# TheProParadox/3dspa_code

Hardware: AMD Instinct MI355X
Metric: train-step tracks/sec (B x N_tracks) at T=150, C=772 (higher is better)
Workload: dtype bf16

## Files before the change

### 3dspa_code_amd/csrc/common.hpp

```cpp
#pragma once
#include <hip/hip_runtime.h>
#include <stdint.h>
#include <string>
#include <vector>

#include "../../include/spa3d.h"
#include "ablate.inc"
#include "gemm_plan.hpp"
#include "score_row.hpp"

#ifndef SPA_F16
#define SPA_F16 0
#endif
#if SPA_F16
#define SPA_NS h_f16
#else
#define SPA_NS h_bf16
#endif
typedef unsigned short bf16_t;

struct DetCfg { float* gbase; long long* shadow; long long n; unsigned* flag; float scale; };
constexpr float DET_ADDEND_MAX = 36028797018963968.f;
constexpr long long DET_SUM_MAX = 1ll << 62;
constexpr int DET_E_MIN = -24, DET_E_MAX = 40;
// ... 117 lines not shown
  bool dry = false, overflow = false;
  void* alloc(int64_t bytes) {
    int64_t a = (off + 255) & ~int64_t(255);
    off = a + bytes;
    if (off > peak) peak = off;
    if (dry) return (void*)(uintptr_t)(0x1000 + a);
    if (off > cap) { overflow = true; return base; }
    return base + a;
  }
  int64_t mark() const { return off; }
  void release(int64_t m) { off = m; }
};

enum { PROF_GEMM_NT = 0, PROF_GEMM_TN = 1, PROF_GEMM_GENERIC = 2, PROF_ATTN_FWD = 3, PROF_ATTN_BWD = 4, PROF_LN_FWD = 5, PROF_LN_BWD = 6,
       PROF_ATTN_Q1 = 7, PROF_EMBED = 8, PROF_NCLS = 9 };
struct ProfRec { int cls; double flops, bytes; hipEvent_t e0, e1; int64_t tag[4] = {0, 0, 0, 0}; };
struct Prof {
  bool on = false;
  std::vector<hipEvent_t> pool; size_t used = 0;
  std::vector<ProfRec> recs;
  hipEvent_t get() {
    if (used == pool.size()) { hipEvent_t e; if (hipEventCreate(&e) != hipSuccess) return nullptr; pool.push_back(e); }
    return pool[used++];
  }
};

struct spa3d_ctx {
  spa3d_config cfg;
  std::vector<Leaf> leaves;
  int64_t nparams = 0;
  std::string err;
  hipStream_t stream = nullptr;
  Arena ar;
  bool dry = false;
  int hip_err = 0;
  GemmPolicy gemm;
  int attn_impl = 0;
  int chunk = 0;
  int query_chunk = 0;
  int track_chunk = 0;
  int ro_share = 1;
  int prune = 1;
  float loss_scale = 1.f;
  void* grad_ev[2] = {nullptr, nullptr};
  int64_t grad_ev_gen[2] = {0, 0};
  bool last_chunk = false;
  const float* loss_scale_state = nullptr;
  double plan_stats[4] = {0, 0, 0, 0};
  int attn_bwd_mode = 0;
  int qkv_attn = 0;
  int det_grads = 0;
  const DetCfg* det = nullptr;
  std::vector<int32_t> cnt_n, cnt_q; bool has_cnt_n = false, has_cnt_q = false; int cnt_B = 0;
  int poison = 0;
  Prof prof;
};

inline void apply_attn_impl(spa3d_ctx* c, int v) {
  c->attn_impl = v == 1 ? 1 : (v >= 2 ? 2 : 0);
  c->attn_bwd_mode = v == 3 ? 2 : (v == 4 ? 3 : 0);
  c->qkv_attn = v == 6;
}

template <typename F> inline int64_t arena_peak(spa3d_ctx* c, F&& body) {
  const Arena saved = c->ar; const bool sd = c->dry;
  c->ar = Arena(); c->ar.dry = true; c->dry = true;
  body();
  const int64_t peak = c->ar.peak;
  c->ar = saved; c->dry = sd;
  return peak;
}
template <typename F> inline int sized_call(spa3d_ctx* c, const char* what, int64_t need, void* ws, int64_t ws_bytes, void* stream, F&& body) {
  if (!ws || ws_bytes < need) { c->err = std::string(what) + ": workspace too small: need " + std::to_string(need) + " bytes"; return SPA3D_ERR_ARG; }
  c->stream = (hipStream_t)stream; c->dry = false;
  c->ar = Arena(); c->ar.base = (char*)ws; c->ar.cap = ws_bytes;
  body();
  if (c->ar.overflow) { c->err = "internal: arena overflow"; return SPA3D_ERR_WORKSPACE; }
  return c->hip_err ? SPA3D_ERR_HIP : SPA3D_OK;
}
inline bool counts_fit_batch(spa3d_ctx* c, int B) {
  if (c->cnt_B == B) return true;
  c->err = "counts were set for B = " + std::to_string(c->cnt_B) + ", this batch has B = " + std::to_string(B);
  return false;
}
inline const int32_t* checked_query_counts(spa3d_ctx* c, int B, int Q) {
  if (!counts_fit_batch(c, B)) return nullptr;
  for (int i = 0; i < B; ++i)
    if (c->cnt_q[i] < 0 || c->cnt_q[i] > Q) {
      c->err = "query_count[" + std::to_string(i) + "] = " + std::to_string(c->cnt_q[i]) + " is outside [0, Q = " + std::to_string(Q) + "]";
      return nullptr;
    }
  return c->cnt_q.data();
}
template <typename F> inline void for_each_live_span(const int32_t* cq, int64_t B, int64_t Q, F&& f) {
  if (!cq) { f((int64_t)0, B * Q); return; }
  for (int64_t i = 0; i < B; ++i) f(i * Q, (int64_t)cq[i]);
}

struct ProfScope {
  spa3d_ctx* c; ProfRec r; bool on;
  ProfScope(spa3d_ctx* c_, int cls, double flops, double bytes) : c(c_), on(c_->prof.on && !c_->dry) {
    if (!on) return;
    r.cls = cls; r.flops = flops; r.bytes = bytes; r.e0 = c->prof.get(); r.e1 = c->prof.get();
    if (!r.e0 || !r.e1) { on = false; return; }
    (void)hipEventRecord(r.e0, c->stream);
  }
// ... 127 lines not shown
```

### 3dspa_code_amd/csrc/gemm_fast.hip

```cpp
#include "common.hpp"
#include "tn_args.hpp"

namespace SPA_NS {

typedef __attribute__((ext_vector_type(4))) float f32x4;
typedef __attribute__((ext_vector_type(16))) float f32x16;
typedef mfma16x8 bf16x8;
typedef __attribute__((ext_vector_type(4))) unsigned short u16x4;

#define GLDS16(gptr, lptr) \
  __builtin_amdgcn_global_load_lds((const __attribute__((address_space(1))) void*)(gptr), (__attribute__((address_space(3))) void*)(lptr), 16, 0, 0)
#define GLDS16_NT(gptr, lptr) \
  __builtin_amdgcn_global_load_lds((const __attribute__((address_space(1))) void*)(gptr), (__attribute__((address_space(3))) void*)(lptr), 16, 0, 2)

__device__ __forceinline__ void glds16_s(const void* base_uniform, unsigned off, const void* lds_dst) {
  const unsigned l = (unsigned)(uintptr_t)lds_dst;
  asm volatile("s_mov_b32 m0, %2\n\ts_nop 0\n\tglobal_load_lds_dwordx4 %0, %1" ::"v"(off), "s"(base_uniform), "s"(l) : "memory", "m0");
}

struct NtArgs {
  const bf16_t* A; const bf16_t* Bt; void* C;
  int64_t M; int N; int K; int64_t lda, ldb, ldc;
  const float* bias; const bf16_t* aux; bf16_t* pre_out; int epi; int out_f32; int accumulate; float alpha;
  int tiles_m, tiles_n, crow_group, crow_skip;
#if SPA3D_ABL_NT
  int ablate;
#endif
  const bf16_t* A2; int64_t lda2; int K1; const int32_t* arow_idx; const int32_t* crow_idx; const bf16_t* r1_x; const float* r1_w;
  int nt_store;
};

__global__ __launch_bounds__(256, 2) void gemm_nt_kernel(NtArgs g) {
  extern __shared__ __attribute__((aligned(16))) char smem[];
  const int bid = blockIdx.x;
  const int xcd = bid & 7, idx = bid >> 3;
  const int tm = (idx / g.tiles_n) * 8 + xcd, tn = idx % g.tiles_n;
  if (tm >= g.tiles_m) return;
  const int64_t m0 = (int64_t)tm * 128;
  const int n0 = tn * 128;
  const int tid = threadIdx.x, lane = tid & 63, w = tid >> 6;
  const int wm = (w >> 1) * 64, wn = (w & 1) * 64;
  const int fr = lane & 15, fq = lane >> 4;

  const int sr = lane >> 3, scp = lane & 7;
  const int sc = (scp ^ sr) * 8;
  const bf16_t* ga[4]; const bf16_t* gb[4];
#pragma unroll
  for (int i = 0; i < 4; ++i) {
    int row = (w * 4 + i) * 8 + sr;
    int64_t am = m0 + row; if (am > g.M - 1) am = g.M - 1;
    int bn = n0 + row; if (bn > g.N - 1) bn = g.N - 1;
    ga[i] = g.A + am * g.lda + sc;
    gb[i] = g.Bt + (int64_t)bn * g.ldb + sc;
  }
  auto stage = [&](int buf, int kt) {
    char* sa = smem + buf * 32768 + (w * 4) * 1024;
    char* sb = sa + 16384;
#pragma unroll
    for (int i = 0; i < 4; ++i) GLDS16(ga[i] + kt * 64, sa + i * 1024);
#pragma unroll
    for (int i = 0; i < 4; ++i) GLDS16(gb[i] + kt * 64, sb + i * 1024);
  };

  f32x4 acc[4][4];
#pragma unroll
  for (int i = 0; i < 4; ++i)
#pragma unroll
    for (int j = 0; j < 4; ++j) acc[i][j] = f32x4{0.f, 0.f, 0.f, 0.f};

  const int nt = g.K / 64;
  stage(0, 0);
  __syncthreads();
  const int a_off = (wm + fr) * 128, b_off = (wn + fr) * 128;
  const int x0 = ((fq) ^ (fr & 7)) * 16, x1 = ((4 + fq) ^ (fr & 7)) * 16;
  for (int t = 0; t < nt; ++t) {
    const int cur = t & 1;
    if (t + 1 < nt) stage(cur ^ 1, t + 1);
    const char* sa = smem + cur * 32768;
    const char* sb = sa + 16384;
#pragma unroll
    for (int ks = 0; ks < 2; ++ks) {
      const int xo = ks ? x1 : x0;
      bf16x8 af[4], bfr[4];
#pragma unroll
      for (int i = 0; i < 4; ++i) af[i] = *(const bf16x8*)(sa + a_off + i * 2048 + xo);
#pragma unroll
      for (int j = 0; j < 4; ++j) bfr[j] = *(const bf16x8*)(sb + b_off + j * 2048 + xo);
#pragma unroll
      for (int i = 0; i < 4; ++i)
#pragma unroll
        for (int j = 0; j < 4; ++j) acc[i][j] = MFMA16(bfr[j], af[i], acc[i][j]);
    }
    __syncthreads();
  }

  float* cs = (float*)smem;
#pragma unroll
  for (int i = 0; i < 4; ++i)
#pragma unroll
    for (int j = 0; j < 4; ++j) {
      const int row = wm + i * 16 + fr, ch = (wn >> 2) + j * 4 + fq;
      *(f32x4*)(cs + row * 128 + ((ch ^ (row & 31)) << 2)) = acc[i][j];
    }
  __syncthreads();
  const int er = tid >> 4, ec = tid & 15;
  const int gn = n0 + ec * 8;
  if (gn >= g.N) return;
  float b8[8];
#pragma unroll
  for (int r = 0; r < 8; ++r) b8[r] = 0.f;
  if (g.bias) { const float4 b0 = *(const float4*)(g.bias + gn), b1 = *(const float4*)(g.bias + gn + 4);
    b8[0] = b0.x; b8[1] = b0.y; b8[2] = b0.z; b8[3] = b0.w; b8[4] = b1.x; b8[5] = b1.y; b8[6] = b1.z; b8[7] = b1.w; }
#pragma unroll 2
  for (int it = 0; it < 8; ++it) {
    const int row = it * 16 + er;
    const int64_t gm = m0 + row;
    if (gm >= g.M) break;
    int64_t crow = gm;
    if (g.crow_group > 0) crow = gm + (gm / g.crow_group + 1) * (int64_t)g.crow_skip;
    const f32x4 v0 = *(const f32x4*)(cs + row * 128 + (((2 * ec) ^ (row & 31)) << 2));
    const f32x4 v1 = *(const f32x4*)(cs + row * 128 + (((2 * ec + 1) ^ (row & 31)) << 2));
    float v[8] = {v0[0], v0[1], v0[2], v0[3], v1[0], v1[1], v1[2], v1[3]};
#pragma unroll
    for (int r = 0; r < 8; ++r) v[r] = g.alpha * v[r] + b8[r];
    const int64_t ci = crow * g.ldc + gn;
    if (g.pre_out) {
      uint4 p4; unsigned* pp = (unsigned*)&p4;
#pragma unroll
      for (int r = 0; r < 4; ++r) pp[r] = f2bf_pack2(v[2 * r], v[2 * r + 1]);
      *(uint4*)(g.pre_out + ci) = p4;
    }
    if (g.epi == EPI_GELU) {
#pragma unroll
      for (int r = 0; r < 8; ++r) v[r] = gelu_tanh_fast_f(v[r]);
    }
    if (g.aux) {
      const uint4 x4 = *(const uint4*)(g.aux + ci); const unsigned* xp = (const unsigned*)&x4;
#pragma unroll
      for (int r = 0; r < 4; ++r) {
        const float xa = unpack_lo(xp[r]), xb = unpack_hi(xp[r]);
        if (g.epi == EPI_MUL_GELU_GRAD) { v[2 * r] *= gelu_tanh_grad_fast_f(xa); v[2 * r + 1] *= gelu_tanh_grad_fast_f(xb); }
        else { v[2 * r] += xa; v[2 * r + 1] += xb; }
      }
    }
    if (g.out_f32) {
      float4* cp = (float4*)((float*)g.C + ci);
      if (g.accumulate) { const float4 o0 = cp[0], o1 = cp[1];
        v[0] += o0.x; v[1] += o0.y; v[2] += o0.z; v[3] += o0.w; v[4] += o1.x; v[5] += o1.y; v[6] += o1.z; v[7] += o1.w; }
      cp[0] = make_float4(v[0], v[1], v[2], v[3]); cp[1] = make_float4(v[4], v[5], v[6], v[7]);
    } else {
      uint4* cp = (uint4*)((bf16_t*)g.C + ci);
      if (g.accumulate) { const uint4 o4 = *cp; const unsigned* op = (const unsigned*)&o4;
#pragma unroll
        for (int r = 0; r < 4; ++r) { v[2 * r] += unpack_lo(op[r]); v[2 * r + 1] += unpack_hi(op[r]); } }
      uint4 o4; unsigned* op = (unsigned*)&o4;
#pragma unroll
      for (int r = 0; r < 4; ++r) op[r] = f2bf_pack2(v[2 * r], v[2 * r + 1]);
      *cp = o4;
    }
  }
}


__global__ __launch_bounds__(256, 4) void gemm_nt_occ_kernel(NtArgs g) {
  extern __shared__ __attribute__((aligned(16))) char smem[];
  const int bid = blockIdx.x;
  const int xcd = bid & 7, idx = bid >> 3;
  const int tm = (idx / g.tiles_n) * 8 + xcd, tn = idx % g.tiles_n;
  if (tm >= g.tiles_m) return;
  const int64_t m0 = (int64_t)tm * 128;
  const int n0 = tn * 128;
  const int tid = threadIdx.x, lane = tid & 63, w = tid >> 6;
  const int wm = (w >> 1) * 64, wn = (w & 1) * 64;
  const int fr = lane & 15, fq = lane >> 4;
  const int sr = lane >> 3, scp = lane & 7;
  const int sc = (scp ^ sr) * 8;
  const bf16_t* ga[4]; const bf16_t* gb[4];
#pragma unroll
  for (int i = 0; i < 4; ++i) {
    int row = (w * 4 + i) * 8 + sr;
    int64_t am = m0 + row; if (am > g.M - 1) am = g.M - 1;
    int bn = n0 + row; if (bn > g.N - 1) bn = g.N - 1;
    ga[i] = g.A + am * g.lda + sc;
    gb[i] = g.Bt + (int64_t)bn * g.ldb + sc;
  }
  f32x4 acc[4][4];
#pragma unroll
  for (int i = 0; i < 4; ++i)
#pragma unroll
    for (int j = 0; j < 4; ++j) acc[i][j] = f32x4{0.f, 0.f, 0.f, 0.f};
  const int nt = g.K / 64;
  const int a_off = (wm + fr) * 128, b_off = (wn + fr) * 128;
  const int x0 = ((fq) ^ (fr & 7)) * 16, x1 = ((4 + fq) ^ (fr & 7)) * 16;
  char* const sa0 = smem + (w * 4) * 1024; char* const sb0 = sa0 + 16384;
  for (int t = 0; t < nt; ++t) {
#pragma unroll
    for (int i = 0; i < 4; ++i) GLDS16(ga[i] + t * 64, sa0 + i * 1024);
#pragma unroll
    for (int i = 0; i < 4; ++i) GLDS16(gb[i] + t * 64, sb0 + i * 1024);
    __syncthreads();
    const char* sa = smem; const char* sb = smem + 16384;
#pragma unroll
    for (int ks = 0; ks < 2; ++ks) {
      const int xo = ks ? x1 : x0;
      bf16x8 af[4], bfr[4];
#pragma unroll
      for (int i = 0; i < 4; ++i) af[i] = *(const bf16x8*)(sa + a_off + i * 2048 + xo);
#pragma unroll
      for (int j = 0; j < 4; ++j) bfr[j] = *(const bf16x8*)(sb + b_off + j * 2048 + xo);
#pragma unroll
      for (int i = 0; i < 4; ++i)
#pragma unroll
        for (int j = 0; j < 4; ++j) acc[i][j] = MFMA16(bfr[j], af[i], acc[i][j]);
// ... 113 lines not shown
#pragma unroll
  for (int r = 0; r < 4; ++r) op[r] = f2bf_pack2(v[2 * r], v[2 * r + 1]);
  return o4;
}

__device__ __forceinline__ void nt_store4(const NtArgs& g, int64_t gm, int gn, const f32x4& a) {
  if (gm >= g.M || gn >= g.N) return;
  int64_t crow = gm;
  if (g.crow_group > 0) crow = gm + (gm / g.crow_group + 1) * (int64_t)g.crow_skip;
  float vv[4];
#pragma unroll
  for (int r = 0; r < 4; ++r) vv[r] = g.alpha * a[r];
  if (g.bias) { const float4 b4 = *(const float4*)(g.bias + gn); vv[0] += b4.x; vv[1] += b4.y; vv[2] += b4.z; vv[3] += b4.w; }
  const int64_t ci = crow * g.ldc + gn;
  if (g.pre_out) { u16x4 p4;
#pragma unroll
    for (int r = 0; r < 4; ++r) p4[r] = f2bf(vv[r]);
    *(u16x4*)(g.pre_out + ci) = p4; }
  if (g.epi == EPI_GELU) {
#pragma unroll
    for (int r = 0; r < 4; ++r) vv[r] = gelu_tanh_fast_f(vv[r]);
  }
  if (g.aux) {
    const u16x4 x4 = *(const u16x4*)(g.aux + ci);
    if (g.epi == EPI_MUL_GELU_GRAD) {
#pragma unroll
      for (int r = 0; r < 4; ++r) vv[r] *= gelu_tanh_grad_fast_f(bf2f(x4[r]));
    } else {
#pragma unroll
      for (int r = 0; r < 4; ++r) vv[r] += bf2f(x4[r]);
    }
  }
  if (g.out_f32) {
    float4* cp = (float4*)((float*)g.C + ci);
    if (g.accumulate) { const float4 o = *cp; vv[0] += o.x; vv[1] += o.y; vv[2] += o.z; vv[3] += o.w; }
    *cp = make_float4(vv[0], vv[1], vv[2], vv[3]);
  } else {
    u16x4* cp = (u16x4*)((bf16_t*)g.C + ci);
    if (g.accumulate) { const u16x4 o = *cp;
#pragma unroll
      for (int r = 0; r < 4; ++r) vv[r] += bf2f(o[r]); }
    u16x4 o4;
#pragma unroll
    for (int r = 0; r < 4; ++r) o4[r] = f2bf(vv[r]);
    *cp = o4;
  }
}

#if SPA3D_ABL_NT
#define NT_ABLATE_STORES && !g.ablate
#else
#define NT_ABLATE_STORES
#endif
#define NT8P_BAR() do { __builtin_amdgcn_sched_barrier(0); __builtin_amdgcn_s_barrier(); __builtin_amdgcn_sched_barrier(0); } while (0)
#define NT8P_WAIT_VM(n) asm volatile("s_waitcnt vmcnt(%0)" ::"n"(n) : "memory")
#define NT8P_WAIT_LGKM(n) asm volatile("s_waitcnt lgkmcnt(%0)" ::"n"(n) : "memory")

template <int WMT, int WNT, bool COARSE = false, bool EMB = false>
__global__ __launch_bounds__(512, (WMT * WNT <= 8 ? 4 : 2)) void gemm_nt8p_kernel(NtArgs g) {
  constexpr int BM = 32 * WMT, BN = 64 * WNT;
  constexpr int NA = WMT / 4, NB = WNT / 2;
  constexpr int HM = WMT / 2, HN = WNT / 2;
  constexpr int ASLOT = BM * 128, BBUF = BN * 128, BOFF = 3 * ASLOT;
  extern __shared__ __attribute__((aligned(16))) char smem[];
  const int bid = blockIdx.x;
  const int xcd = bid & 7, idx = bid >> 3;
  const int tm = (idx / g.tiles_n) * 8 + xcd, tn = idx % g.tiles_n;
  if (tm >= g.tiles_m) return;
  const int64_t m0 = (int64_t)tm * BM;
  const int n0 = tn * BN;
  const int tid = threadIdx.x, lane = tid & 63;
  const int w = __builtin_amdgcn_readfirstlane(tid >> 6);
  const int wr = w >> 2, wc = w & 3;
  const int fr = lane & 15, fq = lane >> 4;
  const int sr = lane >> 3, scp = lane & 7;
  const int sc = (scp ^ sr) * 8;
  const bf16_t* pa[2][NA]; const bf16_t* pb[2][NB];
  const bf16_t* pa2[2][NA];
  int la[2][NA], lb[2][NB];
#pragma unroll
  for (int h = 0; h < 2; ++h) {
#pragma unroll
    for (int i = 0; i < NA; ++i) {
      const int gi = i * 8 + w, ra = (gi / WMT) * (WMT * 16) + h * (WMT * 8) + (gi % WMT) * 8;
      int64_t am = m0 + ra + sr; if (am > g.M - 1) am = g.M - 1;
      if (EMB && g.arow_idx) am = g.arow_idx[am];
      pa[h][i] = g.A + am * g.lda + sc; la[h][i] = ra * 128;
      pa2[h][i] = (EMB && g.A2) ? g.A2 + am * g.lda2 + sc : nullptr;
    }
#pragma unroll
    for (int i = 0; i < NB; ++i) {
      const int gi = i * 8 + w, rb = (gi / WNT) * (WNT * 16) + h * (WNT * 8) + (gi % WNT) * 8;
      int bn = n0 + rb + sr; if (bn > g.N - 1) bn = g.N - 1;
      pb[h][i] = g.Bt + (int64_t)bn * g.ldb + sc; lb[h][i] = BOFF + rb * 128;
    }
  }
  const bool a_once = g.tiles_n == 1;
  const int k1t = (EMB && g.A2) ? g.K1 / 64 : 0x7fffffff;
  auto stageA = [&](int kt, int slot) {
    char* base = smem + slot * ASLOT;
#pragma unroll
    for (int h = 0; h < 2; ++h)
#pragma unroll
      for (int i = 0; i < NA; ++i) {
        const bf16_t* src = (!EMB || kt < k1t) ? pa[h][i] + kt * 64 : pa2[h][i] + (kt - k1t) * 64;
        if (a_once) GLDS16_NT(src, base + la[h][i]); else GLDS16(src, base + la[h][i]);
      }
  };
// ... 383 lines not shown
      load_ax(0, ax[0]);
#pragma unroll
      for (int p = 0; p < NP; ++p) {
        if (p + 1 < NP) load_ax(p + 1, ax[(p + 1) & 1]);
        stage_pass(p / CS, p % CS);
#pragma unroll
        for (int it = 0; it < 2; ++it) {
          float v[8]; read_item(it, v);
          held[p][it] = nt_compute8_aux(g, v, b8[p % CS][it], ax[p & 1][it]);
        }
        __builtin_amdgcn_wave_barrier();
      }
    }
    idx = next_valid(idx + nslot);
    const bool more = idx < per_xcd;
    if (more) {
      m0 = (int64_t)((idx / g.tiles_n) * 8 + xcd) * BM; n0 = (idx % g.tiles_n) * BN;
      set_tile(m0, n0);
      prologue();
    }
    if constexpr (has_aux) {
      typedef __attribute__((ext_vector_type(4))) unsigned u32x4;
#pragma unroll
      for (int p = 0; p < NP; ++p)
#pragma unroll
        for (int it = 0; it < 2; ++it) {
          const int64_t gm = cm0 + (rbase + (p / CS) * 16 + prow[it]);
          if (pval[it] && gm < g.M NT_ABLATE_STORES) {
            u32x4* cp = (u32x4*)((bf16_t*)g.C + gm * g.ldc + gn_of(p % CS, it));
            const u32x4 o = u32x4{held[p][it].x, held[p][it].y, held[p][it].z, held[p][it].w};
            if (g.nt_store) __builtin_nontemporal_store(o, cp); else *cp = o;
          }
        }
    } else {
#pragma unroll
      for (int p = 0; p < NP; ++p) {
        stage_pass(p / CS, p % CS);
#pragma unroll
        for (int it = 0; it < 2; ++it) {
          float v[8]; read_item(it, v);
          const int64_t gm = cm0 + (rbase + (p / CS) * 16 + prow[it]);
          if (pval[it] && gm < g.M NT_ABLATE_STORES) nt_store8<true, false>(g, gm, gn_of(p % CS, it), v, b8[p % CS][it]);
        }
        __builtin_amdgcn_wave_barrier();
      }
    }
    if (!more) break;
    if (!interior) NT8P_WAIT_VM(0);
    else if (nst_code) NT8P_WAIT_VM(NKT + 4 * NP);
    else NT8P_WAIT_VM(NKT + 2 * NP);
  }
}

void gemm_nt_bf16(spa3d_ctx* c, const GemmDesc& d, GemmKernel k) {
  NtArgs g;
  g.A = (const bf16_t*)d.A; g.Bt = (const bf16_t*)(d.Bt ? d.Bt : d.B); g.C = d.C; g.M = d.M; g.N = d.N; g.K = d.K; g.lda = d.sAm; g.ldb = d.Bt ? d.ldBt : d.sBn; g.ldc = d.sCm;
  g.bias = d.bias; g.aux = (const bf16_t*)d.aux; g.pre_out = (bf16_t*)d.pre_out; g.epi = d.epi; g.out_f32 = d.out_f32; g.accumulate = d.accumulate; g.alpha = d.alpha;
  g.tiles_m = (int)((d.M + 127) / 128); g.tiles_n = (d.N + 127) / 128;
  g.crow_group = d.crow_group; g.crow_skip = d.crow_skip;
  g.A2 = (const bf16_t*)d.A2; g.lda2 = d.sA2m; g.K1 = d.K1; g.arow_idx = d.arow_idx; g.crow_idx = d.crow_idx; g.r1_x = (const bf16_t*)d.r1_x; g.r1_w = d.r1_w;
#if SPA3D_ABL_NT
  { const char* e = getenv("SPA3D_ABLATE"); g.ablate = e ? atoi(e) : 0; }
#endif
  g.nt_store = (!d.out_f32 && (double)d.M * d.N * 2.0 >= 512e6) ? 1 : 0;
  const int64_t blocks = (int64_t)((g.tiles_m + 7) / 8) * 8 * g.tiles_n;
  static bool attr_set = false;
  if (!attr_set) { (void)hipFuncSetAttribute((const void*)gemm_nt_kernel, hipFuncAttributeMaxDynamicSharedMemorySize, 65536); attr_set = true; }
  ProfScope ps(c, PROF_GEMM_NT, 2.0 * (double)d.M * d.N * d.K,
               ((double)d.M * d.K + (double)d.K * d.N + (double)d.M * d.N * (d.out_f32 ? 2.0 : 1.0) * (d.accumulate ? 2.0 : 1.0) + (double)d.M * d.N * ((d.aux ? 1.0 : 0.0) + (d.pre_out ? 1.0 : 0.0))) * 2.0);
  ps.tag(d.M, d.N, d.K, gemm_prof_flags(k, d, 0));
  switch (k) {
    case GemmKernel::NtEmbed: g.nt_store = 0; launch_nt8p<4, 6, true>(c, g); break;
    case GemmKernel::Nt8pp256: {
      NtArgs g2 = g; g2.tiles_m = (int)((g.M + 255) / 256); g2.tiles_n = g.N / 256;
      static bool attrp = false;
      if (!attrp) {
        (void)hipFuncSetAttribute((const void*)gemm_nt8pp_kernel<8, 4, true, false>, hipFuncAttributeMaxDynamicSharedMemorySize, 163840);
        (void)hipFuncSetAttribute((const void*)gemm_nt8pp_kernel<8, 4, true, true>, hipFuncAttributeMaxDynamicSharedMemorySize, 163840);
        attrp = true;
      }
      if (d.aux) gemm_nt8pp_kernel<8, 4, true, true><<<256, 512, 163840, c->stream>>>(g2);
      else gemm_nt8pp_kernel<8, 4, true, false><<<256, 512, 163840, c->stream>>>(g2);
      break;
    }
    case GemmKernel::Nt8pp384: {
      NtArgs g2 = g; g2.tiles_m = (int)((g.M + 127) / 128); g2.tiles_n = g.N / 384;
      static bool attrq = false;
      if (!attrq) {
        (void)hipFuncSetAttribute((const void*)gemm_nt8pp_kernel<4, 6, false, false>, hipFuncAttributeMaxDynamicSharedMemorySize, 163840);
        (void)hipFuncSetAttribute((const void*)gemm_nt8pp_kernel<4, 6, false, true>, hipFuncAttributeMaxDynamicSharedMemorySize, 163840);
        attrq = true;
      }
      if (d.aux) gemm_nt8pp_kernel<4, 6, false, true><<<256, 512, 163840, c->stream>>>(g2);
      else gemm_nt8pp_kernel<4, 6, false, false><<<256, 512, 163840, c->stream>>>(g2);
      break;
    }
    case GemmKernel::Nt8p256: launch_nt8p<8, 4>(c, g); break;
    case GemmKernel::Nt8p384: launch_nt8p<4, 6>(c, g); break;
    case GemmKernel::NtOcc: gemm_nt_occ_kernel<<<(unsigned)blocks, 256, 32768, c->stream>>>(g); break;
    default: gemm_nt_kernel<<<(unsigned)blocks, 256, 65536, c->stream>>>(g); break;
  }
  SPA_LAUNCH_CHECK(c);
}


__device__ __forceinline__ uint2 ds_read_tr16_b64(const void* p) {
  uint2 v;
  const unsigned a = (unsigned)(uintptr_t)p;
  asm volatile("ds_read_b64_tr_b16 %0, %1" : "=v"(v) : "v"(a) : "memory");
  return v;
}
__device__ __forceinline__ int tr_off(int row, int ch) { return 256 * row + 16 * (ch ^ (((row & 3) << 2) | ((row >> 2) & 3))); }

__global__ __launch_bounds__(256, 2) void gemm_tn_kernel(TnArgs g) {
  extern __shared__ __attribute__((aligned(16))) char smem[];
  const int xcd = blockIdx.x & 7; int j = blockIdx.x >> 3;
  const int ntile = g.tiles_i * g.tiles_n;
  const int sp = (j / ntile) * 8 + xcd; j %= ntile;
  if (sp >= g.splits) return;
  const int tn = j % g.tiles_n, ti = j / g.tiles_n;
  const int i0 = ti * 128, n0 = tn * 128;
  const int64_t mbeg = (int64_t)sp * g.rows_per_split;
  int64_t mend = mbeg + g.rows_per_split; if (mend > g.M) mend = g.M;
  const int nt = (int)((mend - mbeg + 63) / 64);
  const int tid = threadIdx.x, lane = tid & 63, w = tid >> 6;
  const int wi = (w >> 1) * 64, wn = (w & 1) * 64;

  const int sr = lane >> 4, scp = lane & 15;
  int acol[4], bcol[4];
#pragma unroll
  for (int q = 0; q < 4; ++q) {
    const int row = w * 16 + q * 4 + sr;
    const int ch = scp ^ (((row & 3) << 2) | ((row >> 2) & 3));
    int ca = i0 + ch * 8; if (ca > g.Ki - 8) ca = g.Ki - 8;
    int cb = n0 + ch * 8; if (cb > g.N - 8) cb = g.N - 8;
    acol[q] = ca; bcol[q] = cb;
  }
  auto stage = [&](int buf, int t) {
    char* sa = smem + buf * 32768 + w * 4096;
    char* sb = sa + 16384;
#pragma unroll
    for (int q = 0; q < 4; ++q) {
      const int64_t m = mbeg + (int64_t)t * 64 + w * 16 + q * 4 + sr;
      const bool ok = m < mend;
      int64_t mb = ok ? m : mend - 1;
      if (g.brow_group > 0) mb = mb + (mb / g.brow_group + 1) * (int64_t)g.brow_skip;
      const bf16_t* pa = ok ? g.A + m * g.lda + acol[q] : g.zero;
      const bf16_t* pb = g.B + mb * g.ldb + bcol[q];
      GLDS16(pa, sa + q * 1024);
      GLDS16(pb, sb + q * 1024);
    }
  };

// ... 321 lines not shown
```

### 3dspa_code_amd/csrc/model.hip

```cpp
#include <algorithm>
#include <cmath>
#include <cstring>
#include <map>

#include "common.hpp"
#include <cstdio>

enum { MODE_FORWARD = 0, MODE_TRAIN = 1, MODE_ENCODE = 2, MODE_DECODE = 3 };

struct RunArgs {
  int mode; const float* P; const spa3d_batch* b; float denom; float* G; int accumulate; float* loss3; spa3d_outputs* out;
  const float* latents_in; float* latents_out; int chunk;
  const int32_t* cn; const int32_t* cq;
  const spa3d_scores* score;
};

namespace SPA_NS {
template <typename T>
void attention_fwd(spa3d_ctx* c, const T* q, const T* k, const T* v, int64_t ldq, int64_t ldk, int64_t ldv, const float* sq,
                   const float* sk, const float* km, int64_t nseq, int Sq, int Sk, int H, int Dh, T* o, float* lse, int impl,
                   const int32_t* seq_off = nullptr, int64_t total_rows = 0);
template <typename T>
void attention_bwd(spa3d_ctx* c, const T* q, const T* k, const T* v, int64_t ldq, int64_t ldk, int64_t ldv, const float* sq,
                   const float* sk, const float* km, int64_t nseq, int Sq, int Sk, int H, int Dh, const T* o, const float* lse, const T* d_o,
// ... 1254 lines not shown
    k_score_rows(h, s);
    if (cq) score_zero_rows(h, scores, row0 + nq, b->Q - nq, To);
  });
  if (scores->sample_stats) k_score_reduce(h, scores->query_stats, b->B, b->Q, scores->num_thresholds, scores->sample_stats);
  return h->hip_err ? SPA3D_ERR_HIP : SPA3D_OK;
}

int spa3d_loss_and_grads(spa3d_handle h, const float* params, const spa3d_batch* b, float denom, float* grads, int32_t accumulate,
                         float* loss3, spa3d_outputs* out, void* ws, int64_t ws_bytes, void* stream) {
  if (!h || !params || !grads) return SPA3D_ERR_ARG;
  if (accumulate && h->loss_scale != 1.f) { h->err = "accumulate=1 is not supported with a loss scale (fp16 mode)"; return SPA3D_ERR_ARG; }
  RunArgs a{}; a.mode = MODE_TRAIN; a.P = params; a.b = b; a.denom = denom; a.G = grads; a.accumulate = accumulate; a.loss3 = loss3; a.out = out;
  return run(h, a, ws, ws_bytes, stream);
}

int spa3d_loss(spa3d_handle h, const spa3d_batch* b, const spa3d_outputs* preds, float denom, float* loss3, void* stream) {
  if (!h || !b || !preds || !loss3 || !preds->tracks || !preds->visible_logits || !b->query_tracks || !b->query_tracks_visible)
    return SPA3D_ERR_ARG;
  h->err.clear(); h->hip_err = 0; h->stream = (hipStream_t)stream; h->dry = false;
  if (((uintptr_t)loss3) & 7) { h->err = "loss3 must be 8-byte aligned"; return SPA3D_ERR_ARG; }
  float* scratch = loss3 + 4;
  unsigned* poison = (unsigned*)(loss3 + 3);
  const int To = h->cfg.num_output_frames, NC = h->cfg.model_kind == 1 ? 2 : 3;
  const int32_t* cq = nullptr;
  if (h->has_cnt_q && !(cq = checked_query_counts(h, b->B, b->Q))) return SPA3D_ERR_ARG;
  k_zero(h, loss3 + 3, 36);
  for_each_live_span(cq, b->B, b->Q, [&](int64_t row0, int64_t nq) { k_vis_count(h, b->query_tracks_visible + row0 * To, nq * To, scratch + 4, poison); });
  k_set_denom(h, scratch, poison, denom, scratch + 6);
  for_each_live_span(cq, b->B, b->Q, [&](int64_t row0, int64_t nq) {
    const int64_t r = row0 * To;
    k_loss_from_preds(h, preds->tracks + r * NC, preds->visible_logits + r, nq * To, b->query_tracks + r * NC, b->query_tracks_visible + r, scratch, poison, NC);
  });
  k_loss_finalize(h, scratch, poison, scratch + 6, L1_WEIGHT, BCE_WEIGHT, loss3);
  return h->hip_err ? SPA3D_ERR_HIP : SPA3D_OK;
}

int spa3d_set_option(spa3d_handle h, const char* name, double value) {
  if (!h || !name) return SPA3D_ERR_ARG;
  const std::string n(name);
  if (n == "prune") h->prune = value != 0;
  else if (n == "ro_share") h->ro_share = value != 0;
  else if (n == "loss_scale") { if (h->cfg.precision != SPA3D_F16) { h->err = "loss_scale applies to SPA3D_F16 handles only"; return SPA3D_ERR_ARG; } h->loss_scale = (float)value; }
  else if (n == "attn_impl") apply_attn_impl(h, (int)value);
  else if (n == "gemm_impl") set_gemm_impl(h, (int)value);
  else if (n == "chunk") {
    if (value > 1 && (h->query_chunk > 0 || h->track_chunk > 0)) { h->err = "\"chunk\" > 1 cannot be combined with \"query_chunk\" / \"track_chunk\""; return SPA3D_ERR_ARG; }
    h->chunk = value > 0 ? (int)value : 0;
  }
  else if (n == "query_chunk" || n == "track_chunk") {
    if (!(value >= 0 && value <= 2147483647.0)) { h->err = n + " must be >= 0"; return SPA3D_ERR_ARG; }
    if (value >= 1 && h->chunk > 1) { h->err = "\"" + n + "\" cannot be combined with \"chunk\" > 1 (it implies one sample per chunk)"; return SPA3D_ERR_ARG; }
    (n == "query_chunk" ? h->query_chunk : h->track_chunk) = (int)value;
  }
  else if (n == "poison") h->poison = value != 0;
  else if (n == "det_grads") h->det_grads = value != 0;
  else { h->err = "unknown option: " + n; return SPA3D_ERR_ARG; }
  return SPA3D_OK;
}
int spa3d_set_loss_scale_state(spa3d_handle h, const float* state) {
  if (!h) return SPA3D_ERR_ARG;
  h->loss_scale_state = state;
  return SPA3D_OK;
}
int spa3d_set_counts(spa3d_handle h, int32_t B, const int32_t* support_count, const int32_t* query_count) {
  if (!h) return SPA3D_ERR_ARG;
  h->has_cnt_n = h->has_cnt_q = false; h->cnt_n.clear(); h->cnt_q.clear(); h->cnt_B = 0;
  if (!support_count && !query_count) return SPA3D_OK;
  if (B <= 0) { h->err = "spa3d_set_counts: B must be positive"; return SPA3D_ERR_ARG; }
  h->cnt_B = B;
  if (support_count) { h->cnt_n.assign(support_count, support_count + B); h->has_cnt_n = true; }
  if (query_count) { h->cnt_q.assign(query_count, query_count + B); h->has_cnt_q = true; }
  return SPA3D_OK;
}
int spa3d_grad_segments(spa3d_handle h, int64_t* bounds4) {
  if (!h || !bounds4) return SPA3D_ERR_ARG;
  int64_t b1 = -1, b2 = -1;
  for (auto& l : h->leaves) {
    if (b1 < 0 && l.name.rfind("tracks_to_latents/", 0) == 0) b1 = l.offset;
    if (b2 < 0 && l.name.rfind("track_readout_attn/", 0) == 0) b2 = l.offset;
  }
  if (b1 < 0 || b2 < b1) return SPA3D_ERR_ARG;
  bounds4[0] = 0; bounds4[1] = b1; bounds4[2] = b2; bounds4[3] = h->nparams;
  return SPA3D_OK;
}
int spa3d_grad_events_recorded(spa3d_handle h, int64_t* out4) {
  if (!h || !out4) return SPA3D_ERR_ARG;
  out4[0] = h->grad_ev_gen[0]; out4[1] = h->grad_ev_gen[1]; out4[2] = (int64_t)(intptr_t)h->grad_ev[0]; out4[3] = (int64_t)(intptr_t)h->grad_ev[1];
  return SPA3D_OK;
}
int spa3d_detach(spa3d_handle h, void* ev_readout, void* ev_latents, const float* loss_scale_state) {
  if (!h) return SPA3D_ERR_ARG;
  if (ev_readout && h->grad_ev[0] == ev_readout && h->grad_ev[1] == ev_latents) { h->grad_ev[0] = nullptr; h->grad_ev[1] = nullptr; }
  if (loss_scale_state && h->loss_scale_state == loss_scale_state) h->loss_scale_state = nullptr;
  return SPA3D_OK;
}
int spa3d_set_grad_events(spa3d_handle h, void* ev_readout, void* ev_latents) {
  if (!h) return SPA3D_ERR_ARG;
  h->grad_ev[0] = ev_readout; h->grad_ev[1] = ev_latents;
  return SPA3D_OK;
}
int spa3d_plan_stats(spa3d_handle h, double* out4) {
  if (!h || !out4) return SPA3D_ERR_ARG;
  for (int i = 0; i < 4; ++i) out4[i] = h->plan_stats[i];
  return SPA3D_OK;
}

// ... 49 lines not shown
```

### 3dspa_code_amd/csrc/ops.hip

```cpp
#include <cmath>

#include "common.hpp"

namespace SPA_NS {
namespace {
struct OpCtx : spa3d_ctx {
  OpCtx(void* stream_, void* ws, int64_t ws_bytes) {
    stream = (hipStream_t)stream_; ar.base = (char*)ws; ar.cap = ws_bytes;
  }
  template <typename U> U* alloc(int64_t n) { return (U*)ar.alloc(n * (int64_t)sizeof(U)); }
  int status() { return ar.overflow ? SPA3D_ERR_WORKSPACE : (hip_err ? SPA3D_ERR_HIP : SPA3D_OK); }
};

template <typename T>
int op_linear(OpCtx& c, const T* A, const T* B, const float* bias, const T* res, T* C, int64_t M, int N, int K, int act, int impl) {
  GemmDesc d{};
  d.A = A; d.B = B; d.C = C; d.M = M; d.N = N; d.K = K; d.sAm = K; d.sAk = 1; d.sBk = N; d.sBn = 1; d.sCm = N;
  d.bias = bias; d.epi = act == 1 ? EPI_GELU : (act == 2 ? EPI_MUL_GELU_GRAD : EPI_NONE); d.aux = res;
  const GemmPolicy p = GemmPolicy::from_impl(impl & 15);
  if constexpr (sizeof(T) == 2) {
    if (p.only != GemmKernel::Refuse) {
      const bool rs = p.only == GemmKernel::Rs;
      const void*& pk = rs ? d.rs_pk : d.ntb_pk;
      pk = A;
      if (plan_nt(d, p) != p.only) return SPA3D_ERR_ARG;
      T* w = c.alloc<T>(rs ? gemm_rs_pack_elems(N) : gemm_ntb_pack_elems(K, N));
      if (c.ar.overflow) return SPA3D_ERR_WORKSPACE;
      if (rs) gemm_rs_pack<T>(&c, B, N, 1, N, w); else gemm_ntb_pack<T>(&c, B, N, 1, K, N, w);
      pk = w;
      if (plan_nt(d, p) != p.only) return SPA3D_ERR_ARG;
      gemm_launch<T>(&c, d, p.only);
      return c.status();
    }
    if (impl != 1) {
      if (impl & 16) { d.pre_out = c.alloc<T>(M * N); if (c.ar.overflow) return SPA3D_ERR_WORKSPACE; }
      T* Bt = c.alloc<T>((int64_t)K * N);
      if (c.ar.overflow) return SPA3D_ERR_WORKSPACE;
      k_transpose<T>(&c, B, K, N, Bt);
      d.Bt = Bt; d.ldBt = K;
      const GemmKernel k = plan_nt(d, GemmPolicy::from_impl((impl & 15) == 1 ? 0 : impl & 15));
      if (k != GemmKernel::Refuse) { gemm_launch<T>(&c, d, k); return c.status(); }
    }
  }
  if ((impl & 15) >= 2) return SPA3D_ERR_ARG;
  gemm_launch<T>(&c, d, GemmKernel::Generic);
  return c.status();
}

template <typename T>
int op_linear_bwd(OpCtx& c, const T* A, const T* B, const T* dC, T* dA, float* dB, float* dbias, int64_t M, int N, int K, int impl) {
  const GemmPolicy p = GemmPolicy::from_impl(impl == 7 ? 2 : impl);
  if (dA) {
    GemmDesc d{};
    d.A = dC; d.B = B; d.C = dA; d.M = M; d.N = K; d.K = N; d.sAm = N; d.sAk = 1; d.sBk = 1; d.sBn = N; d.sCm = K;
    d.Bt = B; d.ldBt = N;
    GemmKernel k = GemmKernel::Refuse;
    if constexpr (sizeof(T) == 2) {
      if (p.only == GemmKernel::Ntb) {
        d.ntb_pk = dC;
        if (plan_nt(d, p) != GemmKernel::Ntb) return SPA3D_ERR_ARG;
        T* pk = c.alloc<T>(gemm_ntb_pack_elems(N, K));
        if (c.ar.overflow) return SPA3D_ERR_WORKSPACE;
        gemm_ntb_pack<T>(&c, B, 1, N, N, K, pk);
        d.ntb_pk = pk;
      }
      k = plan_nt(d, p);
    }
    if (k == GemmKernel::Refuse) { if (impl >= 2) return SPA3D_ERR_ARG; k = GemmKernel::Generic; }
    gemm_launch<T>(&c, d, k);
  }
  if (dB) {
    k_zero(&c, dB, (int64_t)K * N * 4);
    GemmDesc d{};
    d.A = A; d.B = dC; d.C = dB; d.M = K; d.N = N; d.K = M; d.sAm = 1; d.sAk = K; d.sBk = N; d.sBn = 1; d.sCm = N;
    d.out_f32 = 1; d.accumulate = 1;
    void* zp = c.alloc<char>(256); k_zero(&c, zp, 256); d.zero_page = zp;
    GemmKernel k = GemmKernel::Refuse;
    if constexpr (sizeof(T) == 2) k = plan_tn(d, p);
    if (k == GemmKernel::Refuse) { if (impl >= 2) return SPA3D_ERR_ARG; k = GemmKernel::Generic; }
    gemm_launch<T>(&c, d, k);
  }
  if (dbias) { k_zero(&c, dbias, (int64_t)N * 4); k_colsum<T>(&c, dC, M, N, N, dbias); }
  return c.status();
}
}

template <typename T>
void attention_fwd(spa3d_ctx* c, const T* q, const T* k, const T* v, int64_t ldq, int64_t ldk, int64_t ldv, const float* sq,
                   const float* sk, const float* km, int64_t nseq, int Sq, int Sk, int H, int Dh, T* o, float* lse, int impl,
                   const int32_t* seq_off = nullptr, int64_t total_rows = 0);
template <typename T>
void attention_bwd(spa3d_ctx* c, const T* q, const T* k, const T* v, int64_t ldq, int64_t ldk, int64_t ldv, const float* sq,
                   const float* sk, const float* km, int64_t nseq, int Sq, int Sk, int H, int Dh, const T* o, const float* lse, const T* d_o,
                   T* dq, T* dk, T* dv, float* dsq, float* dsk, int impl, const int32_t* seq_off = nullptr, int64_t total_rows = 0);
}

extern "C" {
#pragma GCC visibility push(hidden)
int spa3d_op_sin_embed_f16(const float* x, int64_t rows, int32_t C, int32_t nf, void* out, int32_t dtype, void* stream);
int spa3d_op_linear_f16(const void* A, const void* B, const float* bias, const void* residual, void* C, int64_t M, int32_t N, int32_t K,
                        int32_t act, int32_t dtype, int32_t impl, void* ws, int64_t ws_bytes, void* stream);
int spa3d_op_linear_bwd_f16(const void* A, const void* B, const void* dC, void* dA, float* dB, float* dbias, int64_t M, int32_t N, int32_t K,
                            int32_t dtype, int32_t impl, void* ws, int64_t ws_bytes, void* stream);
int spa3d_op_mlp_fused_f16(const void* na, const void* a, const void* w_in, const float* b_in, const void* w_out, const float* b_out, void* y,
                           void* h, void* hpre, int64_t M, int32_t d, int32_t mlp, int32_t dtype, void* ws, int64_t ws_bytes, void* stream);
int spa3d_op_qkv_attention_f16(const void* nq, int64_t ldn, const void* wq, const void* wk, const void* wv, const float* scale_q, const float* scale_k,
                               const float* keymask, const int32_t* seq_off, int64_t nseq, int32_t S, int32_t H, void* qkv, void* o, float* lse,
                               int32_t dtype, void* ws, int64_t ws_bytes, void* stream);
int spa3d_op_layernorm_f16(const void* x, const float* scale, void* y, float* stats, int64_t rows, int32_t d, int32_t dtype, void* stream);
int spa3d_op_layernorm_bwd_f16(const void* x, const float* scale, const float* stats, const void* dy, void* dx, float* dscale, int64_t rows,
                               int32_t d, int32_t dtype, void* stream);
int spa3d_op_attention_f16(const void* q, const void* k, const void* v, int64_t ldq, int64_t ldk, int64_t ldv, const float* scale_q,
                           const float* scale_k, const float* keymask, int64_t nseq, int32_t Sq, int32_t Sk, int32_t H, int32_t Dh, void* o,
                           float* lse, int32_t dtype, int32_t impl, void* ws, int64_t ws_bytes, void* stream);
int spa3d_op_attention_bwd_f16(const void* q, const void* k, const void* v, int64_t ldq, int64_t ldk, int64_t ldv, const float* scale_q,
                               const float* scale_k, const float* keymask, int64_t nseq, int32_t Sq, int32_t Sk, int32_t H, int32_t Dh,
                               const void* o, const float* lse, const void* d_o, void* dq, void* dk, void* dv, float* dscale_q,
                               float* dscale_k, int32_t dtype, int32_t impl, void* ws, int64_t ws_bytes, void* stream);
#pragma GCC visibility pop
}
#if SPA_F16
#define spa3d_op_sin_embed spa3d_op_sin_embed_f16
#define spa3d_op_linear spa3d_op_linear_f16
#define spa3d_op_linear_bwd spa3d_op_linear_bwd_f16
#define spa3d_op_layernorm spa3d_op_layernorm_f16
#define spa3d_op_mlp_fused spa3d_op_mlp_fused_f16
#define spa3d_op_qkv_attention spa3d_op_qkv_attention_f16
#define spa3d_op_layernorm_bwd spa3d_op_layernorm_bwd_f16
// ... 118 lines not shown
```

Baseline: 92310.

## Add multi-slot LDS ring pipeline to NT GEMM for single-round grids

Templates the NT GEMM tile body on the number of LDS stages and adds a 3- or 4-slot ring variant that prefetches several K tiles ahead, using counted vmcnt waits and raw barriers instead of a full sync per step. By default the ring is chosen for small grids that fit in one round of blocks with enough K tiles, trading occupancy (launch bounds 1, up to 128KB LDS) for deeper memory latency hiding. Also adds op-level flags for fp32/accumulate output and row mapping, plus a gemm_ring option.

```diff
diff --git a/3dspa_code_amd/csrc/common.hpp b/3dspa_code_amd/csrc/common.hpp
--- a/3dspa_code_amd/csrc/common.hpp
+++ b/3dspa_code_amd/csrc/common.hpp
@@ -193,6 +193,7 @@
   int det_grads = 0;
   const DetCfg* det = nullptr;
   std::vector<int32_t> cnt_n, cnt_q; bool has_cnt_n = false, has_cnt_q = false; int cnt_B = 0;
+  int gemm_ring = 0;
   int poison = 0;
   Prof prof;
 };
diff --git a/3dspa_code_amd/csrc/gemm_fast.hip b/3dspa_code_amd/csrc/gemm_fast.hip
--- a/3dspa_code_amd/csrc/gemm_fast.hip
+++ b/3dspa_code_amd/csrc/gemm_fast.hip
@@ -17,6 +17,9 @@
   const unsigned l = (unsigned)(uintptr_t)lds_dst;
   asm volatile("s_mov_b32 m0, %2\n\ts_nop 0\n\tglobal_load_lds_dwordx4 %0, %1" ::"v"(off), "s"(base_uniform), "s"(l) : "memory", "m0");
 }
+
+#define NT8P_BAR() do { __builtin_amdgcn_sched_barrier(0); __builtin_amdgcn_s_barrier(); __builtin_amdgcn_sched_barrier(0); } while (0)
+#define NT8P_WAIT_VM(n) asm volatile("s_waitcnt vmcnt(%0)" ::"n"(n) : "memory")
 
 struct NtArgs {
   const bf16_t* A; const bf16_t* Bt; void* C;
@@ -30,8 +33,16 @@
   int nt_store;
 };
 
-__global__ __launch_bounds__(256, 2) void gemm_nt_kernel(NtArgs g) {
-  extern __shared__ __attribute__((aligned(16))) char smem[];
+template <int LA>
+__device__ __forceinline__ void ring_wait_tile(int rem) {
+  static_assert(LA == 2 || LA == 3, "ring of 3 or 4 slots");
+  if (rem >= LA - 1) NT8P_WAIT_VM(8 * (LA - 1));
+  else if (LA > 2 && rem == 1) NT8P_WAIT_VM(8);
+  else NT8P_WAIT_VM(0);
+}
+
+template <int NS>
+__device__ __forceinline__ void gemm_nt_tile(const NtArgs& g, char* smem) {
   const int bid = blockIdx.x;
   const int xcd = bid & 7, idx = bid >> 3;
   const int tm = (idx / g.tiles_n) * 8 + xcd, tn = idx % g.tiles_n;
@@ -69,14 +80,14 @@
     for (int j = 0; j < 4; ++j) acc[i][j] = f32x4{0.f, 0.f, 0.f, 0.f};
 
   const int nt = g.K / 64;
-  stage(0, 0);
-  __syncthreads();
+  if constexpr (NS == 2) {
+    stage(0, 0);
+    __syncthreads();
+  }
   const int a_off = (wm + fr) * 128, b_off = (wn + fr) * 128;
   const int x0 = ((fq) ^ (fr & 7)) * 16, x1 = ((4 + fq) ^ (fr & 7)) * 16;
-  for (int t = 0; t < nt; ++t) {
-    const int cur = t & 1;
-    if (t + 1 < nt) stage(cur ^ 1, t + 1);
-    const char* sa = smem + cur * 32768;
+  auto mma_tile = [&](int buf) {
+    const char* sa = smem + buf * 32768;
     const char* sb = sa + 16384;
 #pragma unroll
     for (int ks = 0; ks < 2; ++ks) {
@@ -90,6 +101,27 @@
       for (int i = 0; i < 4; ++i)
 #pragma unroll
         for (int j = 0; j < 4; ++j) acc[i][j] = MFMA16(bfr[j], af[i], acc[i][j]);
+    }
+  };
+  if constexpr (NS == 2) {
+    for (int t = 0; t < nt; ++t) {
+      const int cur = t & 1;
+      if (t + 1 < nt) stage(cur ^ 1, t + 1);
+      mma_tile(cur);
+      __syncthreads();
+    }
+  } else {
+    constexpr int LA = NS - 1;
+#pragma unroll
+    for (int t = 0; t < LA; ++t)
+      if (t < nt) stage(t, t);
+    int cur = 0, nxt = LA;
+    for (int t = 0; t < nt; ++t) {
+      ring_wait_tile<LA>(nt - 1 - t);
+      NT8P_BAR();
+      if (t + LA < nt) stage(nxt, t + LA);
+      mma_tile(cur);
+      cur = cur + 1 == NS ? 0 : cur + 1; nxt = nxt + 1 == NS ? 0 : nxt + 1;
     }
     __syncthreads();
   }
@@ -159,6 +191,16 @@
       *cp = o4;
     }
   }
+}
+
+__global__ __launch_bounds__(256, 2) void gemm_nt_kernel(NtArgs g) {
+  extern __shared__ __attribute__((aligned(16))) char smem[];
+  gemm_nt_tile<2>(g, smem);
+}
+template <int NS>
+__global__ __launch_bounds__(256, 1) void gemm_nt_ring_kernel(NtArgs g) {
+  extern __shared__ __attribute__((aligned(16))) char smem[];
+  gemm_nt_tile<NS>(g, smem);
 }
 
 
@@ -378,8 +420,6 @@
 #else
 #define NT_ABLATE_STORES
 #endif
-#define NT8P_BAR() do { __builtin_amdgcn_sched_barrier(0); __builtin_amdgcn_s_barrier(); __builtin_amdgcn_sched_barrier(0); } while (0)
-#define NT8P_WAIT_VM(n) asm volatile("s_waitcnt vmcnt(%0)" ::"n"(n) : "memory")
 #define NT8P_WAIT_LGKM(n) asm volatile("s_waitcnt lgkmcnt(%0)" ::"n"(n) : "memory")
 
 template <int WMT, int WNT, bool COARSE = false, bool EMB = false>
@@ -869,6 +909,18 @@
   }
 }
 
+static int nt_ring_slots(const spa3d_ctx* c, GemmKernel k, int tiles_m, int tiles_n, int ktiles) {
+  const int f = c->gemm_ring & 15;
+  if (f == 1) return 0;
+  if (f == 3 || f == 4) return f;
+  const bool one_round = (int64_t)((tiles_m + 7) / 8) * tiles_n <= 32;
+  return one_round && ktiles >= (k == GemmKernel::NtOcc ? 8 : 4) ? 4 : 0;
+}
+template <typename KernelT>
+static void ring_lds_attr(KernelT* kern, int bytes, bool* done) {
+  if (!*done) { (void)hipFuncSetAttribute((const void*)kern, hipFuncAttributeMaxDynamicSharedMemorySize, bytes); *done = true; }
+}
+
 void gemm_nt_bf16(spa3d_ctx* c, const GemmDesc& d, GemmKernel k) {
   NtArgs g;
   g.A = (const bf16_t*)d.A; g.Bt = (const bf16_t*)(d.Bt ? d.Bt : d.B); g.C = d.C; g.M = d.M; g.N = d.N; g.K = d.K; g.lda = d.sAm; g.ldb = d.Bt ? d.ldBt : d.sBn; g.ldc = d.sCm;
@@ -885,7 +937,8 @@
   if (!attr_set) { (void)hipFuncSetAttribute((const void*)gemm_nt_kernel, hipFuncAttributeMaxDynamicSharedMemorySize, 65536); attr_set = true; }
   ProfScope ps(c, PROF_GEMM_NT, 2.0 * (double)d.M * d.N * d.K,
                ((double)d.M * d.K + (double)d.K * d.N + (double)d.M * d.N * (d.out_f32 ? 2.0 : 1.0) * (d.accumulate ? 2.0 : 1.0) + (double)d.M * d.N * ((d.aux ? 1.0 : 0.0) + (d.pre_out ? 1.0 : 0.0))) * 2.0);
-  ps.tag(d.M, d.N, d.K, gemm_prof_flags(k, d, 0));
+  const int ns = k == GemmKernel::Nt || k == GemmKernel::NtOcc ? nt_ring_slots(c, k, g.tiles_m, g.tiles_n, d.K / 64) : 0;
+  ps.tag(d.M, d.N, d.K, gemm_prof_flags(k, d, 0) | (ns ? 1 << 22 : 0));
   switch (k) {
     case GemmKernel::NtEmbed: g.nt_store = 0; launch_nt8p<4, 6, true>(c, g); break;
     case GemmKernel::Nt8pp256: {
@@ -914,8 +967,14 @@
     }
     case GemmKernel::Nt8p256: launch_nt8p<8, 4>(c, g); break;
     case GemmKernel::Nt8p384: launch_nt8p<4, 6>(c, g); break;
-    case GemmKernel::NtOcc: gemm_nt_occ_kernel<<<(unsigned)blocks, 256, 32768, c->stream>>>(g); break;
-    default: gemm_nt_kernel<<<(unsigned)blocks, 256, 65536, c->stream>>>(g); break;
+    default: {
+      static bool a3 = false, a4 = false;
+      if (ns == 3) { ring_lds_attr(gemm_nt_ring_kernel<3>, 3 * 32768, &a3); gemm_nt_ring_kernel<3><<<(unsigned)blocks, 256, 3 * 32768, c->stream>>>(g); }
+      else if (ns == 4) { ring_lds_attr(gemm_nt_ring_kernel<4>, 4 * 32768, &a4); gemm_nt_ring_kernel<4><<<(unsigned)blocks, 256, 4 * 32768, c->stream>>>(g); }
+      else if (k == GemmKernel::NtOcc) gemm_nt_occ_kernel<<<(unsigned)blocks, 256, 32768, c->stream>>>(g);
+      else gemm_nt_kernel<<<(unsigned)blocks, 256, 65536, c->stream>>>(g);
+      break;
+    }
   }
   SPA_LAUNCH_CHECK(c);
 }
diff --git a/3dspa_code_amd/csrc/model.hip b/3dspa_code_amd/csrc/model.hip
--- a/3dspa_code_amd/csrc/model.hip
+++ b/3dspa_code_amd/csrc/model.hip
@@ -1330,6 +1330,11 @@
     if (value >= 1 && h->chunk > 1) { h->err = "\"" + n + "\" cannot be combined with \"chunk\" > 1 (it implies one sample per chunk)"; return SPA3D_ERR_ARG; }
     (n == "query_chunk" ? h->query_chunk : h->track_chunk) = (int)value;
   }
+  else if (n == "gemm_ring") {
+    const int v = (int)value;
+    if (!(value == 0 || value == 1 || value == 3 || value == 4)) { h->err = "gemm_ring: 0, 1, 3 or 4"; return SPA3D_ERR_ARG; }
+    h->gemm_ring = v;
+  }
   else if (n == "poison") h->poison = value != 0;
   else if (n == "det_grads") h->det_grads = value != 0;
   else { h->err = "unknown option: " + n; return SPA3D_ERR_ARG; }
diff --git a/3dspa_code_amd/csrc/ops.hip b/3dspa_code_amd/csrc/ops.hip
--- a/3dspa_code_amd/csrc/ops.hip
+++ b/3dspa_code_amd/csrc/ops.hip
@@ -12,10 +12,24 @@
   int status() { return ar.overflow ? SPA3D_ERR_WORKSPACE : (hip_err ? SPA3D_ERR_HIP : SPA3D_OK); }
 };
 
+enum { OP_RING_SHIFT = 6, OP_F32 = 256, OP_ACC = 512, OP_ROWMAP = 1024, OP_ROWMAP_GROUP = 150 };
+inline int op_take_ring(OpCtx& c, int impl) {
+  const int r = (impl >> OP_RING_SHIFT) & 3;
+  c.gemm_ring = r <= 1 ? r : r + 1;
+  return impl & ~(3 << OP_RING_SHIFT);
+}
+
 template <typename T>
 int op_linear(OpCtx& c, const T* A, const T* B, const float* bias, const T* res, T* C, int64_t M, int N, int K, int act, int impl) {
+  impl = op_take_ring(c, impl);
   GemmDesc d{};
   d.A = A; d.B = B; d.C = C; d.M = M; d.N = N; d.K = K; d.sAm = K; d.sAk = 1; d.sBk = N; d.sBn = 1; d.sCm = N;
+  if constexpr (sizeof(T) == 2) {
+    d.out_f32 = (impl & OP_F32) != 0; d.accumulate = (impl & OP_ACC) != 0;
+    if (impl & OP_ROWMAP) { d.crow_group = OP_ROWMAP_GROUP; d.crow_skip = 1; }
+  }
+  if ((impl & (OP_F32 | OP_ACC | OP_ROWMAP)) && (impl & 15) != 2) return SPA3D_ERR_ARG;
+  impl &= ~(OP_F32 | OP_ACC | OP_ROWMAP);
   d.bias = bias; d.epi = act == 1 ? EPI_GELU : (act == 2 ? EPI_MUL_GELU_GRAD : EPI_NONE); d.aux = res;
   const GemmPolicy p = GemmPolicy::from_impl(impl & 15);
   if constexpr (sizeof(T) == 2) {
@@ -49,6 +63,10 @@
 
 template <typename T>
 int op_linear_bwd(OpCtx& c, const T* A, const T* B, const T* dC, T* dA, float* dB, float* dbias, int64_t M, int N, int K, int impl) {
+  impl = op_take_ring(c, impl);
+  const bool acc = impl & OP_ACC, rowmap = impl & OP_ROWMAP;
+  if ((acc || rowmap) && (impl & ~(OP_ACC | OP_ROWMAP)) != 2) return SPA3D_ERR_ARG;
+  impl &= ~(OP_ACC | OP_ROWMAP);
   const GemmPolicy p = GemmPolicy::from_impl(impl == 7 ? 2 : impl);
   if (dA) {
     GemmDesc d{};
@@ -70,10 +88,11 @@
     gemm_launch<T>(&c, d, k);
   }
   if (dB) {
-    k_zero(&c, dB, (int64_t)K * N * 4);
+    if (!acc) k_zero(&c, dB, (int64_t)K * N * 4);
     GemmDesc d{};
     d.A = A; d.B = dC; d.C = dB; d.M = K; d.N = N; d.K = M; d.sAm = 1; d.sAk = K; d.sBk = N; d.sBn = 1; d.sCm = N;
     d.out_f32 = 1; d.accumulate = 1;
+    if (rowmap) { d.brow_group = OP_ROWMAP_GROUP; d.brow_skip = 1; }
     void* zp = c.alloc<char>(256); k_zero(&c, zp, 256); d.zero_page = zp;
     GemmKernel k = GemmKernel::Refuse;
     if constexpr (sizeof(T) == 2) k = plan_tn(d, p);
```

New measurement: 92460 (median of 6 runs). About the same (+0.2%).
